# HIPS/DESI-MCMC

Hardware: AMD Instinct MI355X
Metric: source-pixel evals/sec + full-field log-lik ms, 10k sources x 5 bands x 2048^2 (higher is better)
Workload: dtype f64

## Files before the change

### desi-mcmc_amd/csrc/celeste_hip.hip

```cpp

#include <hip/hip_runtime.h>
#include <hip/hip_ext.h>

#include <cmath>
#include <cstdarg>
#include <cstddef>
#include <cstdint>
#include <cstdio>
#include <cstring>
#include <algorithm>
#include <atomic>
#include <memory>
#include <new>
#include <vector>
#include <type_traits>

#include "../../include/celeste_hip.h"
#include "host_buf.h"
#include "field_state.h"

static thread_local char g_err[512] = "";

static int fail(int code, const char *fmt, ...) {
    va_list ap;
// ... 141 lines not shown
    DevBuf<BandDev> d_bands;
    DevBuf<double> d_nelec, d_lambda, d_partials, d_llband;
    bool have_nelec = false;
    DevBuf<double> d_slabs;
    DevBuf<int> d_part_cnt;
    DevBuf<SrcRec> d_recs;
    DevBuf<int4> d_boxes;
    DevBuf<int> d_kind;
    DevBuf<int> d_status;
    DevBuf<unsigned long long> d_massfx;
    DevBuf<int> d_mass_todo;
    std::vector<int4> h_boxes;
    std::vector<int> h_status;
    DevBuf<int> d_tile_cnt, d_tile_nstar, d_tile_work, d_order;
    DevBuf<int> d_tile_cost;
    bool bin_two_level = false;
    DevBuf<long long> d_btot;
    int64_t masked[MAX_BANDS] = {0};
    bool any_masked = false;
    bool star_one_segment = false;
    hipEvent_t ev_step = nullptr;
    DevBuf<int64_t> d_tile_off;
    unsigned long long *d_cursor = nullptr;
    DevBuf<int> d_lists;
    int nsx = 0, nsy = 0;
    DevBuf<int> d_sup_cnt;
    DevBuf<int64_t> d_sup_off;
    DevBuf<int> d_clist;
    DevBuf<unsigned long long> d_timing;
    DevBuf<int> d_samp;
    PinnedBuf<double> h_ssum;
    PinnedBuf<int64_t> h_soff;
    DevBuf<NzEntry> d_nzlist;
    DevBuf<double> d_rate;
    DevBuf<int4> d_sbox;
    DevBuf<int4> d_snz;
    DevBuf<int64_t> d_soff;
    DevBuf<double> d_ssum;
    DevBuf<int> d_nnz, d_nzmode;
    DevBuf<int64_t> d_nzoff;
    DevBuf<double> d_stats;
    DevBuf<char> d_slice;
    std::unique_ptr<cel_sources, SourcesDeleter> slice_prop;
    DevBuf<char> d_sgen;
    std::unique_ptr<cel_sources, SourcesDeleter> sgen_prop;
    double last_entries = 0;
// ... 382 lines not shown
        }
        if (!(im->hb[b].R > 0.0))
            im->hb[b].R = host_bounding_radius(bands[b].mu, bands[b].cov, K_PSF, 0.001, nullptr);
        band_to_dev(im->hb[b], hb[b]);
    }
    im->star_one_segment = true;
    for (int b = 0; b < B; b++)
        for (int k = 0; k < K_PSF; k++) {
            const BandDev &d = hb[b];
            const double inv = 1.0 / (d.cxx[k] * d.cyy[k] - d.cxy[k] * d.cxy[k]);
            const double rb_ = d.R + 2.0;
            const double emax = 0.5 * quad_max_rect_hw(d.cyy[k] * inv, -d.cxy[k] * inv, d.cxx[k] * inv, -rb_ - d.mux[k], rb_ - d.mux[k],
                                                       -rb_ - d.muy[k], rb_ - d.muy[k]);
            if (!(emax <= 0.999 * STAR_EMAX)) im->star_one_segment = false;
        }
    const int64_t npix = (int64_t)B * H * W;
    const int T = B * im->ntx * im->nty, NS = B * im->nsx * im->nsy;
    hipStream_t st = c->stream;
    HIP_TRY(im->d_bands.grow(B, B, st));
    HIP_TRY(hipMemcpy(im->d_bands, hb, sizeof(BandDev) * B, hipMemcpyHostToDevice));
    HIP_TRY(im->d_nelec.grow(npix, npix, st));
    HIP_TRY(im->d_lambda.grow(npix, npix, st));
    HIP_TRY(im->d_partials.grow(T, T, st));
    HIP_TRY(im->d_llband.grow(MAX_BANDS + 4, MAX_BANDS + 4, st));
    im->d_cursor = reinterpret_cast<unsigned long long *>(im->d_llband + MAX_BANDS);
    HIP_TRY(im->d_tile_cnt.grow(T, T, st));
    HIP_TRY(im->d_tile_nstar.grow(T, T, st));
    HIP_TRY(im->d_tile_work.grow(T, T, st));
    HIP_TRY(im->d_tile_cost.grow(T, T, st));
    HIP_TRY(im->d_order.grow(T, T, st));
    HIP_TRY(im->d_tile_off.grow(T, T, st));
    HIP_TRY(im->d_sup_cnt.grow(NS, NS, st));
    HIP_TRY(im->d_sup_off.grow(NS, NS, st));
    HIP_TRY(im->d_stats.grow(2, 2, st));
    HIP_TRY(hipMemsetAsync(im->d_lambda, 0, sizeof(double) * npix, st));
    im->counted = true;
    c->live++;
    *out = im.release();
    return CEL_OK;
}

int cel_images_set_nelec(cel_images *im, const double *nelec, int mem) {
    if (!im || !nelec) return fail(CEL_ERR_INVALID, "cel_images_set_nelec: null argument");
    HIP_TRY(hipSetDevice(im->ctx->device));
    int rc = copy_in(im->d_nelec, nelec, sizeof(double) * (size_t)im->B * im->H * im->W, mem, im->ctx->stream);
    if (rc != CEL_OK) return rc;
    im->have_nelec = true;
    im->new_pixels();
// ... 200 lines not shown
    HIP_TRY(hipMemcpyAsync(d, h.data(), bytes, hipMemcpyHostToDevice, st));
    const double *dd = reinterpret_cast<const double *>(d + ints);
    hipLaunchKernelGGL(k_scatter_rows, dim3((unsigned)((n + 255) / 256)), dim3(256), 0, st, n, B, (const int *)d, (const int *)d + n,
                       dd, dd + 2 * n, dd + (2 + B) * n, s->d_type, s->d_radec, s->d_counts, s->d_shape);
    HIP_TRY(hipGetLastError());
    HIP_TRY(hipStreamSynchronize(st));
    s->rows_replaced(s->S, n, idx, type);
    return CEL_OK;
}

static int ensure_recs(cel_images *im, int64_t n) {
    if (n <= im->d_recs.cap) return CEL_OK;
    im->records_regrown();
    const int64_t cap = n + n / 4 + 64;
    HIP_TRY(grow_group(im->ctx->stream, im->d_boxes, cap, im->d_kind, cap, im->d_status, cap, im->d_recs, cap));
    return CEL_OK;
}

static double rsq_galaxy() {
    double q = 1.0 - 1e-5;
    return -2.0 * log1p(-q);
}

static int run_prep(cel_images *im, cel_sources *src, const int *d_live = nullptr, int nobox = 0) {
    cel_ctx *c = im->ctx;
    int64_t n = src->S * im->B;
    int rc = ensure_recs(im, n > 0 ? n : 1);
    if (rc) return rc;
    if (n == 0) { im->records_written(src->gen, 0); return CEL_OK; }
    int pi = prof_slot(c, CEL_K_PREP);
    LAUNCH_EV(k_prep, dim3((unsigned)((n + 255) / 256)), dim3(256), c->stream, EV0(c, pi), EV1(c, pi), im->d_bands, im->B,
              im->full_H, im->W, im->win_y0, im->H, src->S, src->d_type, src->d_radec, src->d_counts, src->d_shape,
              rsq_galaxy(), im->d_recs, im->d_boxes, im->d_kind, im->d_status, im->d_cursor, d_live, nobox);
    HIP_TRY(hipGetLastError());
    im->records_written((d_live || nobox) ? 0 : src->gen, src->S);
    return CEL_OK;
}

static int host_boxes(cel_images *im, cel_sources *src) {
    if (im->rec.host_boxes_of(*src)) return CEL_OK;
    int rc = im->rec.of(*src) ? CEL_OK : run_prep(im, src);
    if (rc) return rc;
    const int64_t n = src->S * im->B;
    im->h_boxes.resize((size_t)n);
    im->h_status.resize((size_t)n);
    if (n) {
        hipStream_t st = im->ctx->stream;
        HIP_TRY(hipMemcpyAsync(im->h_boxes.data(), im->d_boxes, sizeof(int4) * n, hipMemcpyDeviceToHost, st));
        HIP_TRY(hipMemcpyAsync(im->h_status.data(), im->d_status, sizeof(int) * n, hipMemcpyDeviceToHost, st));
        HIP_TRY(hipStreamSynchronize(st));
    }
    im->host_boxes_read(src->gen);
    return CEL_OK;
}

#define CEL_RENDER_STRICT 4
// ... 38 lines not shown
        int mul = (int)(nblk_band * 0.381966) | 1;
        auto gcd = [](int a, int b) { while (b) { int t = a % b; a = b; b = t; } return a; };
        while (mul > 1 && gcd(mul, nblk_band) != 1) mul += 2;
        if (nblk_band < 4) mul = 1;
        x.perm_mul = mul % nblk_band ? mul % nblk_band : 1;
        x.perm_add = nblk_band / 3 + 1;
    }
    x.stamps = nullptr;
    static const char *stamp_path = getenv("CEL_SMALL_STAMPS");
    DevBuf<unsigned long long> d_stamps;
    if (stamp_path) { HIP_TRY(d_stamps.grow(8 * nblk, 8 * nblk, st)); x.stamps = d_stamps; }
    int pi = prof_slot(c, CEL_K_SMALL_STARS);
    LAUNCH_EV(k_small_stars, dim3((unsigned)nblk), dim3(64 * SMALL_NWV), st, EV0(c, pi), EV1(c, pi), a, x);
    const bool ll = (flags & CEL_RENDER_LOGLIK) != 0;
    HIP_TRY(hipGetLastError());
    HIP_TRY(hipStreamSynchronize(st));
    if (d_stamps) {
        std::vector<unsigned long long> hs((size_t)8 * nblk);
        (void)hipMemcpy(hs.data(), d_stamps, sizeof(unsigned long long) * 8 * nblk, hipMemcpyDeviceToHost);
        if (FILE *fp = fopen(stamp_path, "wb")) { fwrite(hs.data(), sizeof(unsigned long long), hs.size(), fp); fclose(fp); }
    }
    unsigned long long cur0;
    memcpy(&cur0, im->h_small + nblk, sizeof(cur0));
    if (cur0 == x.stamp) { im->small_off = true; return CEL_OK; }
    if (ll) {
        for (int b = 0; b < B; b++) {
            const double *pb = im->h_small + (size_t)b * nblk_band;
            double sum[8] = {0, 0, 0, 0, 0, 0, 0, 0}, comp[8] = {0, 0, 0, 0, 0, 0, 0, 0};
            int i = 0;
            for (; i + 8 <= nblk_band; i += 8)
                for (int k = 0; k < 8; k++) {
                    const double y = pb[i + k] - comp[k];
                    const double t = sum[k] + y;
                    comp[k] = (t - sum[k]) - y;
                    sum[k] = t;
                }
            for (int k = 0; i < nblk_band; i++, k++) {
                const double y = pb[i] - comp[k];
                const double t = sum[k] + y;
                comp[k] = (t - sum[k]) - y;
                sum[k] = t;
            }
            c->mail->ll_band[b] = ((sum[0] + sum[1]) + (sum[2] + sum[3])) + ((sum[4] + sum[5]) + (sum[6] + sum[7]));
            im->h_llband[b] = c->mail->ll_band[b];
        }
        im->llband_on_host = true;
    }
// ... 28 lines not shown
    if (p.own_rows && (flags & CEL_RENDER_LOGLIK)) {
        if (im->noise_y0 % im->TH != 0 || (im->noise_y1 % im->TH != 0 && im->noise_y1 < im->H))
            return fail(CEL_ERR_INVALID, "the owned rows [%d, %d) must begin and end on render-tile rows (%d) for a log-likelihood",
                        im->noise_y0, im->noise_y1, im->TH);
        p.own_ty0 = im->noise_y0 / im->TH;
        p.own_ty1 = std::min(im->nty, (im->noise_y1 + im->TH - 1) / im->TH);
    }
    p.diag = c->tile_timing || (c->debug & ~64);
    const bool stars = im->TW == HW_TW && !p.diag && c->variant != 0 && src->n_gal == 0 && im->star_one_segment;
    p.stars_only = stars && c->star_tiles && (c->star_tiles == 2 || T > STAR_TILES_MIN);
    p.small_stars = stars && S > 0 && S <= SMALL_MAX_S && T <= STAR_TILES_MIN && c->star_tiles == 1 && !im->small_off && !lambda_out &&
                    !p.keep_lists && !(flags & CEL_RENDER_STRICT) && !p.own_rows;
    p.parts = p.diag ? 1 : tile_parts_of(c, im);
    p.parts_used = (im->TW == HW_TW && !p.diag) ? p.parts : 1;
    if (p.stars_only) p.parts_used = 0;
    p.incremental = c->incremental && !lambda_out && !(flags & (CEL_RENDER_NO_STORE | CEL_RENDER_STRICT)) && im->TW == HW_TW &&
                    c->variant != 0 && !p.diag && !p.stars_only && p.parts == 1 && S > 0 &&
                    im->incremental_base(*src, S, c->render_T, (flags & CEL_RENDER_LOGLIK) && !p.masked_ll);
    p.tile_order = tile_order_of(c, im);
    p.bin_direct = S > 0 && S <= BIN_DIRECT_MAX_S && (int64_t)T * S <= ((int64_t)1 << 25);
    return CEL_OK;
}

static void launch_bin_fine(cel_ctx *c, cel_images *im, int64_t S, int NS, bool one_level, hipEvent_t e0, hipEvent_t e1) {
    auto go = [&](auto kernel, int waves) {
        LAUNCH_EV(kernel, dim3(NS), dim3(64 * waves), c->stream, e0, e1,
                  im->d_boxes, im->d_kind, S, im->ntx, im->nty, im->TH, im->TW,
                  im->nsx, im->nsy, im->d_sup_cnt, im->d_sup_off, im->d_clist, im->d_clist.cap, im->d_tile_cnt,
                  im->d_tile_nstar, im->d_tile_work, im->d_tile_off, im->d_cursor, im->d_lists, im->d_lists.cap,
                  (int *)(im->d_cursor + 1), (int *)(im->d_cursor + 3));
    };
    const bool small_blocks = NS > c->n_cu;
    if (!one_level) { if (small_blocks) go(k_bin_fine_blk<false, 8>, 8); else go(k_bin_fine_blk<false, 16>, 16); }
    else { if (small_blocks) go(k_bin_fine_blk<true, 8>, 8); else go(k_bin_fine_blk<true, 16>, 16); }
}

static void launch_render(cel_ctx *c, const cel_images *im, const RenderPlan &p, int T, const RenderArgs &a, hipEvent_t e0, hipEvent_t e1) {
    hipStream_t st = c->stream;
    if (im->TW == QW_TW)
        LAUNCH_EV(k_render_qw, dim3(T), dim3(64), st, e0, e1, a);
    else if (im->TW == HW_TW) {
        if (p.diag) LAUNCH_EV(k_render_hw<true>, dim3(T), dim3(64), st, e0, e1, a);
        else if (p.stars_only) LAUNCH_EV((k_render_stars<2, false>), dim3(T), dim3(64), st, e0, e1, a);
        else if (p.parts > 1) {
            const unsigned grid = (unsigned)(((T + 7) / 8) * 8 * p.parts);
            if (p.parts == 4) LAUNCH_EV((k_render_hw<false, 4>), dim3(grid), dim3(64), st, e0, e1, a);
            else LAUNCH_EV((k_render_hw<false, 2>), dim3(grid), dim3(64), st, e0, e1, a);
        }
        else LAUNCH_EV(k_render_hw<false>, dim3(T), dim3(64), st, e0, e1, a);
    }
    else if (im->TH == 64)
        LAUNCH_EV((k_render<64>), dim3(T), dim3(64), st, e0, e1, a);
    else
// ... 52 lines not shown
            return CEL_OK;
        }
    }
    DeltaRows delta;
    delta.n = 0;
    bool incr = plan.incremental;
    auto mark_dirty = [&] {
        hipLaunchKernelGGL(k_mark_dirty, dim3((unsigned)((delta.n * im->B + 255) / 256)), dim3(256), 0, st, delta, (const int4 *)im->d_boxes, S, im->B,
                           im->ntx, im->nty, im->TW, im->TH, im->d_dirty);
    };
    if (incr) {
        for (int64_t s = 0; s < S && incr; s++)
            if (src->row_gen[(size_t)s] > im->model.lambda_gen) {
                if (delta.n == DELTA_MAX) incr = false;
                else delta.idx[delta.n++] = (int)s;
            }
        if (delta.n == 0) incr = false;
    }
    if (incr) {
        HIP_TRY(im->d_dirty.grow(T, T, st));
        HIP_TRY(hipMemsetAsync(im->d_dirty, 0, sizeof(int) * (size_t)T, st));
        mark_dirty();
    }
    im->render_begins((flags & CEL_RENDER_LOGLIK) != 0, !lambda_out && !(flags & CEL_RENDER_NO_STORE));
    rc = run_prep(im, src);
    if (rc) return rc;
    if (incr) mark_dirty();
    if (im->d_lists.cap == 0) {
        const int64_t n = (S * im->B) * 6 + 1024;
        HIP_TRY(im->d_lists.grow(n, n, st));
    }
    if (im->d_clist.cap == 0) {
        const int64_t n = (S * im->B) * 3 + 1024;
        HIP_TRY(im->d_clist.grow(n, n, st));
    }
    const int NS = im->B * im->nsx * im->nsy;
    const int tile_order = plan.tile_order, parts = plan.parts;
    const bool bin_direct = plan.bin_direct, diag = plan.diag;
    if (bin_direct) HIP_TRY(im->d_lists.grow((int64_t)T * S, (int64_t)T * S, st));
    for (int attempt = 0; attempt < 8; attempt++) {
        if (attempt > 0 || S * im->B == 0) HIP_TRY(hipMemsetAsync(im->d_cursor, 0, sizeof(unsigned long long) * 4, st));
        int pi = prof_slot(c, CEL_K_BIN);
        const bool order_ready = tile_order == 1 && im->lists.order_ready(S);
        const hipEvent_t bin_ev1 = (tile_order && !order_ready) ? (hipEvent_t) nullptr : EV1(c, pi);
        if (bin_direct) {
            LAUNCH_EV(k_bin_direct, dim3(T), dim3(64), st, EV0(c, pi), bin_ev1, im->d_boxes, im->d_kind, S, im->ntx, im->nty, im->TH, im->TW,
                      im->d_tile_cnt, im->d_tile_nstar, im->d_tile_work, im->d_tile_off, im->d_cursor, im->d_lists);
        } else if (im->bin_two_level) {
            LAUNCH_EV(k_bin_coarse, dim3(NS), dim3(64 * COARSE_WAVES), st, EV0(c, pi), (hipEvent_t) nullptr, im->d_boxes, S, im->nsx, im->nsy,
                      im->d_sup_cnt, im->d_sup_off, im->d_cursor + 2, im->d_clist, im->d_clist.cap, (int *)(im->d_cursor + 3));
            launch_bin_fine(c, im, S, NS, false, (hipEvent_t) nullptr, bin_ev1);
        } else {
            launch_bin_fine(c, im, S, NS, true, EV0(c, pi), bin_ev1);
        }
        if (tile_order && !order_ready)
            LAUNCH_EV(k_order, dim3(1), dim3(1024), st, (hipEvent_t) nullptr, EV1(c, pi),
                      (const int *)((im->lists.costs_of(S) && tile_order == 1) ? im->d_tile_cost : im->d_tile_work), T, im->d_order);
        RenderArgs a;
        a.bands = im->d_bands; a.recs = im->d_recs; a.lists = im->d_lists; a.tile_cnt = im->d_tile_cnt;
        a.tile_nstar = im->d_tile_nstar;
        a.tile_off = im->d_tile_off; a.nelec = im->d_nelec; a.lambda = lambda_out ? lambda_out : im->d_lambda; a.partials = im->d_partials;
        a.S = S; a.capacity = im->d_lists.cap; a.B = im->B; a.H = im->H; a.W = im->W; a.ntx = im->ntx; a.nty = im->nty;
        a.flags = (plan.masked_ll ? (flags & ~CEL_RENDER_LOGLIK) : flags) | (c->debug << 8); a.variant = c->variant; a.tail_T = c->render_T; a.order = tile_order ? im->d_order : nullptr;
        a.timing = nullptr;
        a.dirty = incr ? im->d_dirty : nullptr;
        a.cost = (im->TW == HW_TW || im->TW == QW_TW) ? im->d_tile_cost : nullptr;
        if (c->tile_timing) {
            HIP_TRY(im->d_timing.grow(3 * T, 3 * T, st));
            a.timing = im->d_timing;
        }
        a.slabs = nullptr; a.part_cnt = nullptr;
        if (parts > 1) {
            const int64_t slabs = (int64_t)HW_TH * HW_TW * T * parts;
            HIP_TRY(im->d_slabs.grow(slabs, slabs, st));
            if (!im->d_part_cnt) {
                HIP_TRY(im->d_part_cnt.grow(T, T, st));
// ... 14 lines not shown
                               hipMemcpyDeviceToHost, st));
        HIP_TRY(hipGetLastError());
        const bool post_order = (tile_order == 1 && a.cost != nullptr);
        if (post_order) {
            if (!im->ev_step) HIP_TRY(hipEventCreateWithFlags(&im->ev_step, hipEventDisableTiming));
            HIP_TRY(hipEventRecord(im->ev_step, st));
            hipLaunchKernelGGL(k_order, dim3(1), dim3(1024), 0, st, (const int *)im->d_tile_cost, T, im->d_order);
            HIP_TRY(hipEventSynchronize(im->ev_step));
        } else {
            HIP_TRY(hipStreamSynchronize(st));
        }
        const unsigned long long *fine = c->mail->bin_fine, *coarse = c->mail->sh.bin_coarse;
        const bool fine_ok = (fine[1] & 0xffffffffull) == 0 && (int64_t)fine[0] <= im->d_lists.cap;
        const bool too_dense = (coarse[1] & 2ull) != 0;
        const bool coarse_ok = (coarse[1] & 0xffffffffull) == 0 && (int64_t)coarse[0] <= im->d_clist.cap;
        if (coarse_ok) im->last_entries = (double)fine[0];
        if (fine_ok && coarse_ok) {
            im->render_succeeded(*src, S, a.cost != nullptr, post_order,
                                 !lambda_out && !(flags & (CEL_RENDER_NO_STORE | CEL_RENDER_STRICT)) && im->TW == HW_TW && c->variant != 0,
                                 c->render_T, diag ? 0 : plan.parts_used, (flags & CEL_RENDER_LOGLIK) && !plan.masked_ll, incr);
            break;
        }
        im->render_overflowed();
        if (too_dense) { im->bin_two_level = true; continue; }
        const int64_t nc = (int64_t)coarse[0] + (int64_t)coarse[0] / 4 + 1024, nf = (int64_t)fine[0] + (int64_t)fine[0] / 4 + 1024;
        if (!coarse_ok) HIP_TRY(im->d_clist.grow(nc, nc, st));
        if (!fine_ok) HIP_TRY(im->d_lists.grow(nf, nf, st));
        if (attempt == 7) return fail(CEL_ERR_HIP, "tile lists kept overflowing");
    }
    if (flags & CEL_RENDER_LOGLIK) ll_from_mailbox(c, im->B, ll_band, ll_total);
    return CEL_OK;
}

int cel_debug_split_rates(cel_images *im, double *out) {
    if (!im || !out) return fail(CEL_ERR_INVALID, "cel_debug_split_rates: null argument");
    if (!im->d_rate) return fail(CEL_ERR_INVALID, "no totals image: cel_photon_split on the recurrence kernels has not run");
    HIP_TRY(hipSetDevice(im->ctx->device));
    return copy_out(out, im->split.rate_in_lambda ? im->d_lambda : im->d_rate, sizeof(double) * (size_t)im->B * im->H * im->W, CEL_HOST, im->ctx->stream);
}

int cel_debug_last_render(cel_images *im, int64_t *dirty_tiles) {
    if (!im || !dirty_tiles) return fail(CEL_ERR_INVALID, "cel_debug_last_render: null argument");
    *dirty_tiles = -1;
    if (im->model.last_dirty == -1 || !im->d_dirty) return CEL_OK;
    HIP_TRY(hipSetDevice(im->ctx->device));
    const int T = im->B * im->ntx * im->nty;
    std::vector<int> h((size_t)T);
    int rc = copy_out(h.data(), im->d_dirty, sizeof(int) * (size_t)T, CEL_HOST, im->ctx->stream);
    if (rc) return rc;
    int64_t n = 0;
// ... 1505 lines not shown
```

### desi-mcmc_amd/csrc/field_state.h

```cpp
#pragma once
#include <atomic>
#include <cstddef>
#include <cstdint>
#include <vector>

inline std::atomic<uint64_t> g_source_gen{0};

struct SourceStamps {
    uint64_t gen = 0;
    uint64_t uid = 0;
    uint64_t full_gen = 0;
    std::vector<uint64_t> row_gen;
    int64_t n_gal = -1;
    std::vector<int32_t> h_type;

    void created() { uid = ++g_source_gen; }
    void all_rows_changed(bool types_unknown) {
        gen = full_gen = ++g_source_gen;
        row_gen.clear();
        if (types_unknown) { n_gal = -1; h_type.clear(); }
    }
    void rows_replaced(int64_t S, int64_t n, const int32_t *idx, const int32_t *type) {
        if ((int64_t)h_type.size() == S) {
            for (int64_t i = 0; i < n; i++) {
// ... 5 lines not shown
        }
        gen = ++g_source_gen;
        if ((int64_t)row_gen.size() != S) row_gen.assign((size_t)S, 0);
        for (int64_t i = 0; i < n; i++) row_gen[idx[i]] = gen;
    }
    void types_known(const int32_t *type, int64_t S) {
        h_type.assign(type, type + S);
        n_gal = 0;
        for (int64_t i = 0; i < S; i++) n_gal += (type[i] != 0);
    }
};

struct RecordStamps {
    uint64_t recs_gen = 0, hbox_gen = 0;
    int64_t last_S = 0;
    bool of(const SourceStamps &src) const { return src.gen != 0 && recs_gen == src.gen; }
    bool host_boxes_of(const SourceStamps &src) const { return of(src) && hbox_gen == src.gen; }
};

struct ListStamps {
    uint64_t lists_gen = 0;
    int64_t cost_S = -1;
    int64_t order_S = -1;
    bool costs_of(int64_t S) const { return cost_S == S; }
    bool order_ready(int64_t S) const { return order_S == S && cost_S == S; }
};

struct ModelStamps {
    uint64_t lambda_gen = 0;
    uint64_t lambda_uid = 0;
    double lambda_T = -1.0;
    int lambda_parts = 0;
    uint64_t partials_gen = 0;
    int64_t last_dirty = -1;
};

struct SplitStamps {
    int64_t samp_S = 0, samp_total = 0;
    bool ssum_valid = false;
    bool hsum_valid = false;
    bool nz_valid = false;
    bool rate_in_lambda = false;
    uint64_t split_epoch = 0;
    uint64_t massfx_gen = 0;
    double massfx_T = -1.0;
    bool resident_of(int64_t S) const { return samp_S > 0 && samp_S == S; }
// ... 24 lines not shown
    RecordStamps rec;
    ListStamps lists;
    ModelStamps model;
    SplitStamps split;
    PendingMass mass;
    bool nelec_u16 = false;
    bool nelec_shared = false;

    bool model_current(const SourceStamps &src, double render_T) const {
        return src.gen != 0 && model.lambda_gen == src.gen && model.lambda_T == render_T && lists.lists_gen == src.gen &&
               rec.recs_gen == src.gen;
    }
    bool incremental_base(const SourceStamps &src, int64_t S, double render_T, bool need_partials) const {
        return S == rec.last_S && model.lambda_gen != 0 && model.lambda_uid == src.uid && model.lambda_T == render_T &&
               model.lambda_parts == 1 && model.lambda_gen != src.gen && model.lambda_gen >= src.full_gen &&
               lists.lists_gen == model.lambda_gen && rec.recs_gen == model.lambda_gen && (int64_t)src.row_gen.size() == S &&
               (!need_partials || (model.partials_gen == model.lambda_gen && !nelec_shared));
    }

    void new_pixels() { model.partials_gen = 0; split.drop(); nelec_u16 = false; }
    void pixel_range(bool u16) { nelec_u16 = u16; }
    void pixels_handed_out() { nelec_u16 = false; nelec_shared = true; model.partials_gen = 0; }
    void new_sky_level() { model.lambda_gen = 0; model.partials_gen = 0; }
    void new_window() { rec.recs_gen = rec.hbox_gen = 0; model.lambda_gen = lists.lists_gen = 0; split.drop(); }
    void records_regrown() { rec.recs_gen = rec.hbox_gen = 0; }
    void records_written(uint64_t gen, int64_t S) { rec.recs_gen = gen; rec.last_S = S; }
    void host_boxes_read(uint64_t gen) { rec.hbox_gen = gen; }
    void small_star_render(uint64_t gen, int64_t S, bool stored) {
        rec.recs_gen = gen; rec.last_S = S;
        lists.lists_gen = 0; lists.cost_S = lists.order_S = -1;
        if (stored) model.lambda_gen = 0;
    }
    void render_begins(bool loglik, bool stores) {
        if (loglik) model.partials_gen = 0;
        lists.lists_gen = 0;
        if (stores) model.lambda_gen = 0;
        model.last_dirty = -1;
    }
    void render_succeeded(const SourceStamps &src, int64_t S, bool costs, bool ordered, bool vouches, double render_T, int parts,
                          bool partials, bool incremental) {
        lists.cost_S = costs ? S : -1; lists.order_S = ordered ? S : -1;
        lists.lists_gen = src.gen;
        if (vouches) {
            model.lambda_gen = src.gen; model.lambda_uid = src.uid; model.lambda_T = render_T; model.lambda_parts = parts;
            model.partials_gen = partials ? src.gen : 0;
        }
        if (incremental) model.last_dirty = -2;
    }
    void render_overflowed() { lists.cost_S = lists.order_S = -1; }
    void partials_overwritten() { model.partials_gen = 0; }
    void split_begins(bool hw) {
        split.split_epoch++;
        if (hw) split.massfx_gen = 0; else model.partials_gen = 0;
    }
    void split_laid_out(int64_t S, int64_t total, bool sums_by_kernel) {
        split.samp_S = S; split.samp_total = total;
        split.ssum_valid = sums_by_kernel;
        split.hsum_valid = split.nz_valid = false;
    }
    void split_totals_from_model(bool yes) { split.rate_in_lambda = yes; }
    void split_ends(bool host_sums, uint64_t stamp_sums_gen, double tail_T) {
        if (host_sums) split.hsum_valid = true;
        if (stamp_sums_gen) { split.massfx_gen = stamp_sums_gen; split.massfx_T = tail_T; }
    }
    void split_lists_built() { split.nz_valid = true; }
};
```

### desi-mcmc_amd/csrc/k_bin2.h

```cpp
#pragma once
#include "device_common.h"

#define SUPER_W 256
#define SUPER_H 256

__device__ inline bool box_hits(int4 q, int X0, int X1, int Y0, int Y1) {
    return (q.x < X1) && (q.y > X0) && (q.z < Y1) && (q.w > Y0) && (q.y > q.x) && (q.w > q.z);
}

#define COARSE_WAVES 16
__global__ void __launch_bounds__(64 * COARSE_WAVES)
k_bin_coarse(const int4 *__restrict__ boxes, int64_t S, int nsx, int nsy, int *__restrict__ sup_cnt,
             int64_t *__restrict__ sup_off, unsigned long long *cursor, int *__restrict__ clist,
             int64_t capacity, int *overflow) {
    __shared__ int wcnt[COARSE_WAVES];
    __shared__ long long base_s;
    const int st = blockIdx.x;
    const int per_band = nsx * nsy;
    const int b = st / per_band;
    const int t = st - b * per_band;
    const int sy = t / nsx, sx = t - sy * nsx;
    const int X0 = sx * SUPER_W, X1 = X0 + SUPER_W, Y0 = sy * SUPER_H, Y1 = Y0 + SUPER_H;
    const int4 *bx = boxes + (int64_t)b * S;
    const int wave = threadIdx.x >> 6, lane = threadIdx.x & 63;
    const int64_t per = ((S + 64 * COARSE_WAVES - 1) / (64 * COARSE_WAVES)) * 64;
    const int64_t lo = per * wave, hi = (lo + per < S) ? lo + per : S;
    int count = 0;
    for (int64_t s0 = lo; s0 < hi; s0 += 64) {
        int64_t s = s0 + lane;
        bool hit = (s < hi) && box_hits(bx[s], X0, X1, Y0, Y1);
        count += __popcll(__ballot(hit));
    }
    if (lane == 0) wcnt[wave] = count;
    __syncthreads();
    if (threadIdx.x == 0) {
        int tot = 0;
        for (int w = 0; w < COARSE_WAVES; w++) tot += wcnt[w];
// ... 6 lines not shown
    int64_t at0 = base_s;
    for (int w = 0; w < wave; w++) at0 += wcnt[w];
    int run = 0;
    for (int64_t s0 = lo; s0 < hi; s0 += 64) {
        int64_t s = s0 + lane;
        bool hit = (s < hi) && box_hits(bx[s], X0, X1, Y0, Y1);
        unsigned long long m = __ballot(hit);
        if (hit) {
            int64_t at = at0 + run + __popcll(m & ((1ull << lane) - 1ull));
            if (at < capacity) clist[at] = (int)s; else *overflow = 1;
        }
        run += __popcll(m);
    }
}

#define BIN_CH 1024

template <bool FUSED, int FINE_WAVES >
__global__ void __launch_bounds__(64 * FINE_WAVES)
k_bin_fine_blk(const int4 *__restrict__ boxes, const int *__restrict__ kind, int64_t S, int ntx, int nty, int TH,
               int TW, int nsx, int nsy, const int *__restrict__ sup_cnt, const int64_t *__restrict__ sup_off,
               const int *__restrict__ clist, int64_t ccap, int *__restrict__ tile_cnt, int *__restrict__ tile_nstar,
               int *__restrict__ tile_work, int64_t *__restrict__ tile_off, unsigned long long *cursor,
               int *__restrict__ lists, int64_t capacity, int *overflow, int *coarse_overflow) {
    constexpr int BIN_TPW = 32 / FINE_WAVES;
    __shared__ int4 sbox[BIN_CH];
    __shared__ int skind[BIN_CH];
    __shared__ int sid[BIN_CH];
    __shared__ int stcnt[FINE_WAVES * BIN_TPW], stoff[FINE_WAVES * BIN_TPW];
    __shared__ long long sbase;
    const int st = blockIdx.x;
    const int per_band_s = nsx * nsy;
    const int b = st / per_band_s;
    const int t = st - b * per_band_s;
    const int sy = t / nsx, sx = t - sy * nsx;
    const int wave = threadIdx.x >> 6, lane = threadIdx.x & 63;
    const int tpx = SUPER_W / TW, tpy = SUPER_H / TH;
    const int4 *bx = boxes + (int64_t)b * S;
    const int *kd = kind + (int64_t)b * S;
    int n = 0;
    int64_t coff = 0;
    if (FUSED) {
        __shared__ int wcnt[FINE_WAVES];
        const int SX0 = sx * SUPER_W, SX1 = SX0 + SUPER_W, SY0 = sy * SUPER_H, SY1 = SY0 + SUPER_H;
        const int64_t per = ((S + 64 * FINE_WAVES - 1) / (64 * FINE_WAVES)) * 64;
        const int64_t lo = per * wave, hi = (lo + per < S) ? lo + per : S;
        constexpr int SCAN_U = 8;
// ... 111 lines not shown
                const int tl = wave + FINE_WAVES * j;
                if (tl >= tpx * tpy) continue;
                base[j] = sbase + stoff[tl];
                const int tx = sx * tpx + (tl % tpx), ty = sy * tpy + (tl / tpx);
                if (tx >= ntx || ty >= nty) continue;
                const int tile = (b * nty + ty) * ntx + tx;
                int w = work[j];
                for (int o = 32; o > 0; o >>= 1) w += __shfl_down(w, o);
                if (lane == 0) {
                    tile_cnt[tile] = cnt[j];
                    tile_nstar[tile] = nst[j];
                    tile_work[tile] = w;
                    tile_off[tile] = base[j];
                }
            }
        }
    }
}

#define BIN_DIRECT_MAX_S 4096
__global__ void __launch_bounds__(64)
k_bin_direct(const int4 *__restrict__ boxes, const int *__restrict__ kind, int64_t S, int ntx, int nty, int TH, int TW,
             int *__restrict__ tile_cnt, int *__restrict__ tile_nstar, int *__restrict__ tile_work, int64_t *__restrict__ tile_off,
             unsigned long long *cursor, int *__restrict__ lists) {
    const int tile = blockIdx.x, lane = threadIdx.x;
    const int per_band = ntx * nty;
    const int b = tile / per_band;
    const int t = tile - b * per_band;
    const int ty = t / ntx, tx = t - ty * ntx;
    const int X0 = tx * TW, X1 = X0 + TW, Y0 = ty * TH, Y1 = Y0 + TH;
    const int4 *bx = boxes + (int64_t)b * S;
    const int *kd = kind + (int64_t)b * S;
    const int64_t base = (int64_t)tile * S;
    constexpr int U = 8;
    int cnt = 0, nst = 0, work = 0;
    for (int64_t s0 = 0; s0 < S; s0 += 64 * U) {
        int4 q[U];
        int k[U];
#pragma unroll
        for (int u = 0; u < U; u++) {
            const int64_t s = min(s0 + 64 * u + lane, S - 1);
            q[u] = bx[s];
            k[u] = kd[s];
        }
#pragma unroll
        for (int u = 0; u < U; u++) {
            const bool hit = (s0 + 64 * u + lane < S) && box_hits(q[u], X0, X1, Y0, Y1);
// ... 40 lines not shown
```

### desi-mcmc_amd/csrc/k_prep_bin.h

```cpp
#pragma once
#include "device_common.h"
__device__ inline void dev_pixel2equa(const BandDev &b, double x, double y, double cphi, double &ra,
                                      double &dec) {
    double d0 = x - b.rho[0], d1 = y - b.rho[1];
    double i0 = b.ups[0] * d0 + b.ups[1] * d1;
    double i1 = b.ups[2] * d0 + b.ups[3] * d1;
    ra = i0 / cphi + b.phi[0];
    dec = i1 + b.phi[1];
}

__device__ inline double clampd(double v, double lo, double hi) { return fmin(fmax(v, lo), hi); }

__device__ inline double comp_radius(double cxx, double cxy, double cyy, double rsq_inv, double dist) {
    double s1 = sqrt(cxx), s2 = sqrt(cyy);
    double rho = cxy / (s1 * s2);
    double A11 = s1, A21 = rho * s2, A22 = s2 * sqrt(1.0 - rho * rho);
    double An = rsq_inv * (1.0 / (A11 * A11) + (A21 * A21) / (A22 * A22));
    double Bn = rsq_inv * (-2.0 * A21 / (A11 * (A22 * A22)));
    double Cn = rsq_inv * 1.0 / (A22 * A22);
    double maj = 1.0 / sqrt(0.5 * (An + Cn - sqrt(Bn * Bn + (An - Cn) * (An - Cn))));
    return maj + dist;
}

__device__ __forceinline__ void prep_pixel(const BandDev &bd, double ra, double dec, double cphi, double &px, double &py) {
// ... 24 lines not shown
        r.x0 = r.x1 = r.y0 = r.y1 = 0;
        if (r.type >= 0) r.type = -1 - r.type;
    }
}

__device__ __forceinline__ void prep_store(const SrcRec &r, int64_t i, SrcRec *__restrict__ recs, int4 *__restrict__ boxes,
                                           int *__restrict__ kind, int *__restrict__ status) {
    recs[i] = r;
    boxes[i] = make_int4(r.x0, r.x1, r.y0, r.y1);
    kind[i] = r.type < 0 ? 0 : (r.type == 0 ? K_PSF : K_GAL);
    status[i] = r.type >= 0 ? 1 : (r.type == -3 ? -1 : 0);
}

struct PrepArgs {
    const BandDev *bands;
    int B, H, W, win_y0, win_h;
    int64_t S;
    const int *type;
    const double *counts, *shape;
    double rsq_gal;
    SrcRec *recs; int4 *boxes; int *kind; int *status;
    int nobox;
};
__device__ __forceinline__ void prep_one(const BandDev *__restrict__ bands, int b, int64_t s, int64_t i, int B, int H, int W, int win_y0, int win_h,
                                         const int *__restrict__ type, double ra, double dec, const double *__restrict__ counts,
                                         const double *__restrict__ shape, double rsq_gal, SrcRec *__restrict__ recs,
                                         int4 *__restrict__ boxes, int *__restrict__ kind, int *__restrict__ status, int nobox) {
    const BandDev &bd = bands[b];
    SrcRec r;
    memset(&r, 0, sizeof(r));
    int t = type[s];
    double cphi = cos(bd.phi[1] / 180.0 * PI_D);
    double px, py;
    prep_pixel(bd, ra, dec, cphi, px, py);
    r.px = px; r.py = py;
    r.scale = counts[s * B + b];
    r.type = t;
    const double BIG = 1073741824.0;
    if (t == 0) {
        prep_star_box(bd, px, py, H, W, r);
    } else if (t == 1) {
        double theta = shape[4 * s], sig = shape[4 * s + 1], phi_s = shape[4 * s + 2], rho_s = shape[4 * s + 3];
        double ra0, dec0, rax, decx, ray, decy;
        dev_pixel2equa(bd, px, py, cphi, ra0, dec0);
        dev_pixel2equa(bd, px + 10.0, py, cphi, rax, decx);
        dev_pixel2equa(bd, px, py + 10.0, cphi, ray, decy);
        double cosd = cos(dec0 * (PI_D / 180.0));
        double cd0 = (rax - ra0) / 10.0 * cosd, cd1 = (ray - ra0) / 10.0 * cosd;
        double cd2 = (decx - dec0) / 10.0, cd3 = (decy - dec0) / 10.0;
        double phi = (90.0 - phi_s) * PI_D / 180.0;
        double re_deg = fmax(1.0 / 30, sig) / 3600.0;
        double cp = cos(phi), sp = sin(phi);
// ... 34 lines not shown
        double rsq_inv = 1.0 / rsq_gal;
        double bound = -INFINITY;
        for (int k = 0; k < K_PSF; k++) {
            double dist = sqrt(bd.mux[k] * bd.mux[k] + bd.muy[k] * bd.muy[k]);
            for (int j = 0; j < K_PROF; j++) {
                if ((j < K_EXP) ? (theta == 0.0) : (theta == 1.0)) continue;
                double v = c_prof_var[j];
                bound = fmax(bound, comp_radius(v * w00 + bd.cxx[k], v * w01 + bd.cxy[k], v * w11 + bd.cyy[k],
                                                rsq_inv, dist));
            }
        }
        if (!(bound == bound) || !(px == px) || !(py == py)) {
            r.type = -1;
        } else {
            int lx = (int)clampd(px - bound, -BIG, BIG), hx = (int)clampd(px + bound + 1, -BIG, BIG);
            int ly = (int)clampd(py - bound, -BIG, BIG), hy = (int)clampd(py + bound + 1, -BIG, BIG);
            r.x0 = max(0, lx); r.x1 = min(hx, W);
            r.y0 = max(0, ly); r.y1 = min(hy, H);
        }
    } else {
        r.type = -1;
    }
    prep_window(r, py, win_y0, win_h);
    prep_store(r, i, recs, boxes, kind, status);
}

__global__ void __launch_bounds__(256)
k_prep(const BandDev *__restrict__ bands, int B, int H, int W, int win_y0, int win_h, int64_t S,
       const int *__restrict__ type, const double *__restrict__ radec,
       const double *__restrict__ counts, const double *__restrict__ shape, double rsq_gal,
       SrcRec *__restrict__ recs, int4 *__restrict__ boxes, int *__restrict__ kind, int *__restrict__ status,
       unsigned long long *__restrict__ cursor ,
       const int *__restrict__ live ,
       int nobox = 0 ) {
    int64_t i = (int64_t)blockIdx.x * blockDim.x + threadIdx.x;
    if (i < 4 && cursor) cursor[i] = 0ull;
    if (i >= S * B) return;
    int b = (int)(i / S);
    int64_t s = i - (int64_t)b * S;
    if (live && live[s] < 0) return;
    prep_one(bands, b, s, i, B, H, W, win_y0, win_h, type, radec[2 * s], radec[2 * s + 1], counts, shape, rsq_gal, recs, boxes, kind, status, nobox);
}

__global__ void k_set_eps(BandDev *__restrict__ bands, int band, double eps) { bands[band].eps = eps; }

__global__ void __launch_bounds__(256)
k_mixture_params(int64_t N, const double *__restrict__ Wm , const double *__restrict__ v_s ,
                 const double *__restrict__ iw, const double *__restrict__ im, const double *__restrict__ ic, int Kp,
                 const double *__restrict__ amp, const double *__restrict__ sigs, int J,
                 double *__restrict__ weights, double *__restrict__ means, double *__restrict__ covars) {
    const int64_t i = (int64_t)blockIdx.x * blockDim.x + threadIdx.x;
    const int K = Kp * J;
    if (i >= N * K) return;
    const int64_t n = i / K;
    const int c = (int)(i - n * K);
    const int k = c / J, j = c - k * J;
    weights[i] = iw[k] * amp[j];
    means[2 * i + 0] = v_s[2 * n + 0] + im[2 * k + 0];
    means[2 * i + 1] = v_s[2 * n + 1] + im[2 * k + 1];
#pragma unroll
    for (int q = 0; q < 4; q++) covars[4 * i + q] = ic[4 * k + q] + sigs[j] * Wm[4 * n + q];
}

__global__ void k_stats(const SrcRec *__restrict__ recs, int64_t n, double *out) {
// ... 41 lines not shown
```

Before: 365.4 billion.

## Skip re-binning when no source box or kind changed since last render

In incremental mode, the prep kernel compares each source's new bounding box and kind with the stored ones. When anything differs it writes the current step number into one of 32 padded change flags. The coarse, fine and direct binning kernels read these flags at entry and return early when nothing changed, restoring the saved cursor words so the previous tile lists stay valid. New state tracking (binned_S) invalidates this whenever records, lists or the bin form are regrown or changed. It saves the binning work on MCMC steps that do not move boxes, but adds the cost of reading the old boxes in prep and a block-wide reduction at each bin kernel launch.

Measured after the change: 375.8 billion, median of 6. 1.03x the previous value.

```diff
diff --git a/desi-mcmc_amd/csrc/celeste_hip.hip b/desi-mcmc_amd/csrc/celeste_hip.hip
--- a/desi-mcmc_amd/csrc/celeste_hip.hip
+++ b/desi-mcmc_amd/csrc/celeste_hip.hip
@@ -187,6 +187,7 @@
     hipEvent_t ev_step = nullptr;
     DevBuf<int64_t> d_tile_off;
     unsigned long long *d_cursor = nullptr;
+    unsigned long long bin_step = 0;
     DevBuf<int> d_lists;
     int nsx = 0, nsy = 0;
     DevBuf<int> d_sup_cnt;
@@ -615,8 +616,9 @@
     HIP_TRY(im->d_nelec.grow(npix, npix, st));
     HIP_TRY(im->d_lambda.grow(npix, npix, st));
     HIP_TRY(im->d_partials.grow(T, T, st));
-    HIP_TRY(im->d_llband.grow(MAX_BANDS + 4, MAX_BANDS + 4, st));
+    HIP_TRY(im->d_llband.grow(MAX_BANDS + BIN_WORDS, MAX_BANDS + BIN_WORDS, st));
     im->d_cursor = reinterpret_cast<unsigned long long *>(im->d_llband + MAX_BANDS);
+    HIP_TRY(hipMemsetAsync(im->d_cursor, 0, sizeof(unsigned long long) * BIN_WORDS, st));
     HIP_TRY(im->d_tile_cnt.grow(T, T, st));
     HIP_TRY(im->d_tile_nstar.grow(T, T, st));
     HIP_TRY(im->d_tile_work.grow(T, T, st));
@@ -863,7 +865,7 @@
     return -2.0 * log1p(-q);
 }
 
-static int run_prep(cel_images *im, cel_sources *src, const int *d_live = nullptr, int nobox = 0) {
+static int run_prep(cel_images *im, cel_sources *src, const int *d_live = nullptr, int nobox = 0, unsigned long long step = 0) {
     cel_ctx *c = im->ctx;
     int64_t n = src->S * im->B;
     int rc = ensure_recs(im, n > 0 ? n : 1);
@@ -872,7 +874,7 @@
     int pi = prof_slot(c, CEL_K_PREP);
     LAUNCH_EV(k_prep, dim3((unsigned)((n + 255) / 256)), dim3(256), c->stream, EV0(c, pi), EV1(c, pi), im->d_bands, im->B,
               im->full_H, im->W, im->win_y0, im->H, src->S, src->d_type, src->d_radec, src->d_counts, src->d_shape,
-              rsq_galaxy(), im->d_recs, im->d_boxes, im->d_kind, im->d_status, im->d_cursor, d_live, nobox);
+              rsq_galaxy(), im->d_recs, im->d_boxes, im->d_kind, im->d_status, im->d_cursor, (d_live || nobox) ? 0ull : step, d_live, nobox);
     HIP_TRY(hipGetLastError());
     im->records_written((d_live || nobox) ? 0 : src->gen, src->S);
     return CEL_OK;
@@ -957,7 +959,7 @@
     }
     unsigned long long cur0;
     memcpy(&cur0, im->h_small + nblk, sizeof(cur0));
-    if (cur0 == x.stamp) { im->small_off = true; return CEL_OK; }
+    if (cur0 == x.stamp) { im->small_off = true; im->records_written(0, S); return CEL_OK; }
     if (ll) {
         for (int b = 0; b < B; b++) {
             const double *pb = im->h_small + (size_t)b * nblk_band;
@@ -1032,13 +1034,13 @@
     return CEL_OK;
 }
 
-static void launch_bin_fine(cel_ctx *c, cel_images *im, int64_t S, int NS, bool one_level, hipEvent_t e0, hipEvent_t e1) {
+static void launch_bin_fine(cel_ctx *c, cel_images *im, int64_t S, int NS, bool one_level, hipEvent_t e0, hipEvent_t e1, const BinStep &bs) {
     auto go = [&](auto kernel, int waves) {
         LAUNCH_EV(kernel, dim3(NS), dim3(64 * waves), c->stream, e0, e1,
                   im->d_boxes, im->d_kind, S, im->ntx, im->nty, im->TH, im->TW,
                   im->nsx, im->nsy, im->d_sup_cnt, im->d_sup_off, im->d_clist, im->d_clist.cap, im->d_tile_cnt,
                   im->d_tile_nstar, im->d_tile_work, im->d_tile_off, im->d_cursor, im->d_lists, im->d_lists.cap,
-                  (int *)(im->d_cursor + 1), (int *)(im->d_cursor + 3));
+                  (int *)(im->d_cursor + 1), (int *)(im->d_cursor + 3), bs);
     };
     const bool small_blocks = NS > c->n_cu;
     if (!one_level) { if (small_blocks) go(k_bin_fine_blk<false, 8>, 8); else go(k_bin_fine_blk<false, 16>, 16); }
@@ -1137,10 +1139,12 @@
         HIP_TRY(hipMemsetAsync(im->d_dirty, 0, sizeof(int) * (size_t)T, st));
         mark_dirty();
     }
+    bool bins_stand = c->incremental && im->lists.binning_of(S);
     im->render_begins((flags & CEL_RENDER_LOGLIK) != 0, !lambda_out && !(flags & CEL_RENDER_NO_STORE));
-    rc = run_prep(im, src);
+    rc = run_prep(im, src, nullptr, 0, bins_stand ? ++im->bin_step : 0ull);
     if (rc) return rc;
     if (incr) mark_dirty();
+    const int64_t lists_cap0 = im->d_lists.cap, clist_cap0 = im->d_clist.cap;
     if (im->d_lists.cap == 0) {
         const int64_t n = (S * im->B) * 6 + 1024;
         HIP_TRY(im->d_lists.grow(n, n, st));
@@ -1153,20 +1157,22 @@
     const int tile_order = plan.tile_order, parts = plan.parts;
     const bool bin_direct = plan.bin_direct, diag = plan.diag;
     if (bin_direct) HIP_TRY(im->d_lists.grow((int64_t)T * S, (int64_t)T * S, st));
+    if (im->d_lists.cap != lists_cap0 || im->d_clist.cap != clist_cap0) { im->lists_regrown(); bins_stand = false; }
     for (int attempt = 0; attempt < 8; attempt++) {
+        const BinStep bs = {im->d_cursor, im->bin_step, (bins_stand && attempt == 0) ? 0 : 1};
         if (attempt > 0 || S * im->B == 0) HIP_TRY(hipMemsetAsync(im->d_cursor, 0, sizeof(unsigned long long) * 4, st));
         int pi = prof_slot(c, CEL_K_BIN);
         const bool order_ready = tile_order == 1 && im->lists.order_ready(S);
         const hipEvent_t bin_ev1 = (tile_order && !order_ready) ? (hipEvent_t) nullptr : EV1(c, pi);
         if (bin_direct) {
             LAUNCH_EV(k_bin_direct, dim3(T), dim3(64), st, EV0(c, pi), bin_ev1, im->d_boxes, im->d_kind, S, im->ntx, im->nty, im->TH, im->TW,
-                      im->d_tile_cnt, im->d_tile_nstar, im->d_tile_work, im->d_tile_off, im->d_cursor, im->d_lists);
+                      im->d_tile_cnt, im->d_tile_nstar, im->d_tile_work, im->d_tile_off, im->d_cursor, im->d_lists, bs);
         } else if (im->bin_two_level) {
             LAUNCH_EV(k_bin_coarse, dim3(NS), dim3(64 * COARSE_WAVES), st, EV0(c, pi), (hipEvent_t) nullptr, im->d_boxes, S, im->nsx, im->nsy,
-                      im->d_sup_cnt, im->d_sup_off, im->d_cursor + 2, im->d_clist, im->d_clist.cap, (int *)(im->d_cursor + 3));
-            launch_bin_fine(c, im, S, NS, false, (hipEvent_t) nullptr, bin_ev1);
+                      im->d_sup_cnt, im->d_sup_off, im->d_cursor + 2, im->d_clist, im->d_clist.cap, (int *)(im->d_cursor + 3), bs);
+            launch_bin_fine(c, im, S, NS, false, (hipEvent_t) nullptr, bin_ev1, bs);
         } else {
-            launch_bin_fine(c, im, S, NS, true, EV0(c, pi), bin_ev1);
+            launch_bin_fine(c, im, S, NS, true, EV0(c, pi), bin_ev1, bs);
         }
         if (tile_order && !order_ready)
             LAUNCH_EV(k_order, dim3(1), dim3(1024), st, (hipEvent_t) nullptr, EV1(c, pi),
@@ -1227,10 +1233,11 @@
             break;
         }
         im->render_overflowed();
-        if (too_dense) { im->bin_two_level = true; continue; }
+        if (too_dense) { im->bin_two_level = true; im->bin_form_changed(); continue; }
         const int64_t nc = (int64_t)coarse[0] + (int64_t)coarse[0] / 4 + 1024, nf = (int64_t)fine[0] + (int64_t)fine[0] / 4 + 1024;
         if (!coarse_ok) HIP_TRY(im->d_clist.grow(nc, nc, st));
         if (!fine_ok) HIP_TRY(im->d_lists.grow(nf, nf, st));
+        im->lists_regrown();
         if (attempt == 7) return fail(CEL_ERR_HIP, "tile lists kept overflowing");
     }
     if (flags & CEL_RENDER_LOGLIK) ll_from_mailbox(c, im->B, ll_band, ll_total);
diff --git a/desi-mcmc_amd/csrc/field_state.h b/desi-mcmc_amd/csrc/field_state.h
--- a/desi-mcmc_amd/csrc/field_state.h
+++ b/desi-mcmc_amd/csrc/field_state.h
@@ -51,6 +51,8 @@
     uint64_t lists_gen = 0;
     int64_t cost_S = -1;
     int64_t order_S = -1;
+    int64_t binned_S = -1;
+    bool binning_of(int64_t S) const { return S > 0 && binned_S == S; }
     bool costs_of(int64_t S) const { return cost_S == S; }
     bool order_ready(int64_t S) const { return order_S == S && cost_S == S; }
 };
@@ -121,13 +123,13 @@
     void pixel_range(bool u16) { nelec_u16 = u16; }
     void pixels_handed_out() { nelec_u16 = false; nelec_shared = true; model.partials_gen = 0; }
     void new_sky_level() { model.lambda_gen = 0; model.partials_gen = 0; }
-    void new_window() { rec.recs_gen = rec.hbox_gen = 0; model.lambda_gen = lists.lists_gen = 0; split.drop(); }
-    void records_regrown() { rec.recs_gen = rec.hbox_gen = 0; }
-    void records_written(uint64_t gen, int64_t S) { rec.recs_gen = gen; rec.last_S = S; }
+    void new_window() { rec.recs_gen = rec.hbox_gen = 0; model.lambda_gen = lists.lists_gen = 0; lists.binned_S = -1; split.drop(); }
+    void records_regrown() { rec.recs_gen = rec.hbox_gen = 0; lists.binned_S = -1; }
+    void records_written(uint64_t gen, int64_t S) { rec.recs_gen = gen; rec.last_S = S; lists.binned_S = -1; }
     void host_boxes_read(uint64_t gen) { rec.hbox_gen = gen; }
     void small_star_render(uint64_t gen, int64_t S, bool stored) {
         rec.recs_gen = gen; rec.last_S = S;
-        lists.lists_gen = 0; lists.cost_S = lists.order_S = -1;
+        lists.lists_gen = 0; lists.cost_S = lists.order_S = -1; lists.binned_S = -1;
         if (stored) model.lambda_gen = 0;
     }
     void render_begins(bool loglik, bool stores) {
@@ -139,14 +141,16 @@
     void render_succeeded(const SourceStamps &src, int64_t S, bool costs, bool ordered, bool vouches, double render_T, int parts,
                           bool partials, bool incremental) {
         lists.cost_S = costs ? S : -1; lists.order_S = ordered ? S : -1;
-        lists.lists_gen = src.gen;
+        lists.lists_gen = src.gen; lists.binned_S = S;
         if (vouches) {
             model.lambda_gen = src.gen; model.lambda_uid = src.uid; model.lambda_T = render_T; model.lambda_parts = parts;
             model.partials_gen = partials ? src.gen : 0;
         }
         if (incremental) model.last_dirty = -2;
     }
-    void render_overflowed() { lists.cost_S = lists.order_S = -1; }
+    void render_overflowed() { lists.cost_S = lists.order_S = -1; lists.binned_S = -1; }
+    void lists_regrown() { lists.binned_S = -1; }
+    void bin_form_changed() { lists.binned_S = -1; }
     void partials_overwritten() { model.partials_gen = 0; }
     void split_begins(bool hw) {
         split.split_epoch++;
diff --git a/desi-mcmc_amd/csrc/k_bin2.h b/desi-mcmc_amd/csrc/k_bin2.h
--- a/desi-mcmc_amd/csrc/k_bin2.h
+++ b/desi-mcmc_amd/csrc/k_bin2.h
@@ -1,5 +1,6 @@
 #pragma once
 #include "device_common.h"
+#include "k_prep_bin.h"
 
 #define SUPER_W 256
 #define SUPER_H 256
@@ -12,7 +13,8 @@
 __global__ void __launch_bounds__(64 * COARSE_WAVES)
 k_bin_coarse(const int4 *__restrict__ boxes, int64_t S, int nsx, int nsy, int *__restrict__ sup_cnt,
              int64_t *__restrict__ sup_off, unsigned long long *cursor, int *__restrict__ clist,
-             int64_t capacity, int *overflow) {
+             int64_t capacity, int *overflow, BinStep bs) {
+    if (bin_unchanged(bs)) return;
     __shared__ int wcnt[COARSE_WAVES];
     __shared__ long long base_s;
     const int st = blockIdx.x;
@@ -65,7 +67,8 @@
                int TW, int nsx, int nsy, const int *__restrict__ sup_cnt, const int64_t *__restrict__ sup_off,
                const int *__restrict__ clist, int64_t ccap, int *__restrict__ tile_cnt, int *__restrict__ tile_nstar,
                int *__restrict__ tile_work, int64_t *__restrict__ tile_off, unsigned long long *cursor,
-               int *__restrict__ lists, int64_t capacity, int *overflow, int *coarse_overflow) {
+               int *__restrict__ lists, int64_t capacity, int *overflow, int *coarse_overflow, BinStep bs) {
+    if (bin_unchanged(bs)) return;
     constexpr int BIN_TPW = 32 / FINE_WAVES;
     __shared__ int4 sbox[BIN_CH];
     __shared__ int skind[BIN_CH];
@@ -223,7 +226,8 @@
 __global__ void __launch_bounds__(64)
 k_bin_direct(const int4 *__restrict__ boxes, const int *__restrict__ kind, int64_t S, int ntx, int nty, int TH, int TW,
              int *__restrict__ tile_cnt, int *__restrict__ tile_nstar, int *__restrict__ tile_work, int64_t *__restrict__ tile_off,
-             unsigned long long *cursor, int *__restrict__ lists) {
+             unsigned long long *cursor, int *__restrict__ lists, BinStep bs) {
+    if (bin_unchanged(bs)) return;
     const int tile = blockIdx.x, lane = threadIdx.x;
     const int per_band = ntx * nty;
     const int b = tile / per_band;
diff --git a/desi-mcmc_amd/csrc/k_prep_bin.h b/desi-mcmc_amd/csrc/k_prep_bin.h
--- a/desi-mcmc_amd/csrc/k_prep_bin.h
+++ b/desi-mcmc_amd/csrc/k_prep_bin.h
@@ -70,12 +70,10 @@
     SrcRec *recs; int4 *boxes; int *kind; int *status;
     int nobox;
 };
-__device__ __forceinline__ void prep_one(const BandDev *__restrict__ bands, int b, int64_t s, int64_t i, int B, int H, int W, int win_y0, int win_h,
-                                         const int *__restrict__ type, double ra, double dec, const double *__restrict__ counts,
-                                         const double *__restrict__ shape, double rsq_gal, SrcRec *__restrict__ recs,
-                                         int4 *__restrict__ boxes, int *__restrict__ kind, int *__restrict__ status, int nobox) {
+__device__ __forceinline__ void prep_record(const BandDev *__restrict__ bands, int b, int64_t s, int B, int H, int W, int win_y0, int win_h,
+                                            const int *__restrict__ type, double ra, double dec, const double *__restrict__ counts,
+                                            const double *__restrict__ shape, double rsq_gal, int nobox, SrcRec &r) {
     const BandDev &bd = bands[b];
-    SrcRec r;
     memset(&r, 0, sizeof(r));
     int t = type[s];
     double cphi = cos(bd.phi[1] / 180.0 * PI_D);
@@ -156,7 +154,33 @@
         r.type = -1;
     }
     prep_window(r, py, win_y0, win_h);
+}
+__device__ __forceinline__ void prep_one(const BandDev *__restrict__ bands, int b, int64_t s, int64_t i, int B, int H, int W, int win_y0, int win_h,
+                                         const int *__restrict__ type, double ra, double dec, const double *__restrict__ counts,
+                                         const double *__restrict__ shape, double rsq_gal, SrcRec *__restrict__ recs,
+                                         int4 *__restrict__ boxes, int *__restrict__ kind, int *__restrict__ status, int nobox) {
+    SrcRec r;
+    prep_record(bands, b, s, B, H, W, win_y0, win_h, type, ra, dec, counts, shape, rsq_gal, nobox, r);
     prep_store(r, i, recs, boxes, kind, status);
+}
+
+#define BIN_KEEP 4
+#define BIN_LINE 16
+#define BIN_CHANGED 16
+#define BIN_NCHANGED 32
+#define BIN_WORDS (BIN_CHANGED + BIN_LINE * BIN_NCHANGED)
+struct BinStep {
+    unsigned long long *words;
+    unsigned long long step;
+    int force;
+};
+__device__ __forceinline__ bool bin_unchanged(const BinStep &bs) {
+    if (bs.force) return false;
+    int hit = 0;
+    if (threadIdx.x < BIN_NCHANGED) hit = bs.words[BIN_CHANGED + BIN_LINE * threadIdx.x] == bs.step;
+    if (__syncthreads_or(hit)) return false;
+    if (blockIdx.x == 0 && threadIdx.x < 4) bs.words[threadIdx.x] = bs.words[BIN_KEEP + threadIdx.x];
+    return true;
 }
 
 __global__ void __launch_bounds__(256)
@@ -164,16 +188,30 @@
        const int *__restrict__ type, const double *__restrict__ radec,
        const double *__restrict__ counts, const double *__restrict__ shape, double rsq_gal,
        SrcRec *__restrict__ recs, int4 *__restrict__ boxes, int *__restrict__ kind, int *__restrict__ status,
-       unsigned long long *__restrict__ cursor ,
+       unsigned long long *cursor ,
+       unsigned long long step ,
        const int *__restrict__ live ,
        int nobox = 0 ) {
     int64_t i = (int64_t)blockIdx.x * blockDim.x + threadIdx.x;
-    if (i < 4 && cursor) cursor[i] = 0ull;
+    if (i < 4 && cursor) { cursor[BIN_KEEP + i] = cursor[i]; cursor[i] = 0ull; }
     if (i >= S * B) return;
     int b = (int)(i / S);
     int64_t s = i - (int64_t)b * S;
     if (live && live[s] < 0) return;
-    prep_one(bands, b, s, i, B, H, W, win_y0, win_h, type, radec[2 * s], radec[2 * s + 1], counts, shape, rsq_gal, recs, boxes, kind, status, nobox);
+    if (!step) {
+        prep_one(bands, b, s, i, B, H, W, win_y0, win_h, type, radec[2 * s], radec[2 * s + 1], counts, shape, rsq_gal, recs, boxes, kind, status, nobox);
+        return;
+    }
+    const int4 was = boxes[i];
+    const int was_kind = kind[i];
+    SrcRec r;
+    prep_record(bands, b, s, B, H, W, win_y0, win_h, type, radec[2 * s], radec[2 * s + 1], counts, shape, rsq_gal, nobox, r);
+    const int now_kind = r.type < 0 ? 0 : (r.type == 0 ? K_PSF : K_GAL);
+    const bool changed = was.x != r.x0 || was.y != r.x1 || was.z != r.y0 || was.w != r.y1 || was_kind != now_kind;
+    const unsigned long long any = __ballot(changed);
+    if (any && (threadIdx.x & 63) == (unsigned)(__ffsll((long long)any) - 1))
+        __hip_atomic_store(cursor + BIN_CHANGED + BIN_LINE * ((i >> 6) & (BIN_NCHANGED - 1)), step, __ATOMIC_RELAXED, __HIP_MEMORY_SCOPE_AGENT);
+    prep_store(r, i, recs, boxes, kind, status);
 }
 
 __global__ void k_set_eps(BandDev *__restrict__ bands, int band, double eps) { bands[band].eps = eps; }
```
